# ctu-vras/monoforce

Measured on AMD Instinct MI355X. Metric: rollout-steps/sec (batch x horizon) on 256x256 terrain, higher is better.
Workload: dtype f32; 1 GPU; c3: B=1024/GPU x T=500 x N=4 contact points, 256x256 grid (res 0.05 m), one shared terrain+friction map (the same on every rank), integrator=odeint-euler (reference default), forward+backward; BASE...; rollouts_per_gpu=1024, rollouts_total=1024, horizon=500, contact_points=4, parallelism=rollout-sharded x1

## Files before the change

monoforce_amd/csrc/rollout_bwd_cp_kernel.h:

```cpp
#pragma once
#include "rollout_bwd_kernel.h"
#include "rollout_cp_common.h"
#include <type_traits>

namespace mf {

enum { kCpEarly = 0, kCpLate = 1, kCpSaved = 2, kCpStream = 3 };
#ifdef MF_STREAM_PROFILE
extern __device__ unsigned long long mf_stream_prof[16];
#define MF_PROF_T(v) const unsigned long long v = __builtin_readcyclecounter()
#define MF_PROF_ACC(name) unsigned long long name = 0
#define MF_PROF_SUM(name, t0) name += __builtin_readcyclecounter() - (t0)
#define MF_PROF_OUT(slot, val) do { if (lane == 0) atomicAdd(&mf_stream_prof[slot], (unsigned long long)(val)); } while (0)
#define MF_PROF_ADD(slot, t0) MF_PROF_OUT(slot, __builtin_readcyclecounter() - (t0))
#else
#define MF_PROF_T(v)
#define MF_PROF_ACC(name)
#define MF_PROF_SUM(name, t0)
#define MF_PROF_OUT(slot, val)
#define MF_PROF_ADD(slot, t0)
#endif
#ifdef MF_NO_WPE
#define MF_STREAM_WPE
#else
#define MF_STREAM_WPE __attribute__((amdgpu_waves_per_eu((MODE == kCpStream && XS_ONLY && sizeof(S) == 4) ? 2 : 1)))
#endif
template <typename S, int INTEG, bool XS_ONLY, bool GCTRL, int MODE, int SLOTS = 6, int BATCH = 3, bool ZMU = false, bool WIN = false, bool ONE1 = false>
__global__ void __launch_bounds__(MODE == kCpStream ? 192 : (WIN ? 512 : 256)) MF_STREAM_WPE
rollout_bwd_cp_kernel(const RolloutBwdArgs<S> a) {
  constexpr bool ODE = INTEG == MF_INTEG_ODEINT_EULER;
  constexpr bool LATE = MODE == kCpLate, STREAM = MODE == kCpStream, SAVED = MODE == kCpSaved || STREAM;
  using namespace cp;
  using M = Mth<S, std::is_same<S, float>::value>;
  using Msk = typename MaskOf<S>::type;
  constexpr unsigned kS = (unsigned)sizeof(S), kC = 2u * kS;
  const int lane = threadIdx.x & 63;
  const int tid = STREAM ? blockIdx.x * 64 + lane : blockIdx.x * blockDim.x + threadIdx.x;
  const int b = tid >> 4;
  __shared__ S win[WIN ? 2 * kWinW * kWinW : 1];
  int wx0 = 0, wy0 = 0;
  unsigned win_flat0 = 0u, win_shift = 0u;
  if constexpr (WIN) {
    static_assert(MODE != kCpStream && sizeof(S) == 4, "the LDS gradient window serves the float32 one-wave forms");
    win_open<S, true>(a, win, (int)((blockIdx.x * blockDim.x) >> 4), &wx0, &wy0);
    __syncthreads();
    win_shift = 31u - (unsigned)__builtin_clz((unsigned)a.H);
    win_flat0 = (unsigned)wy0 + ((unsigned)wx0 << win_shift);
  }
  if (b >= a.B) return;
  const int p = (tid >> 2) & 3, q = tid & 3, cc = q < 3 ? q : 2;
  const S one = S(1.0), zero = S(0.0);
  const int HW = a.H * a.W, last = HW - 1;
  const unsigned moff = a.map_shared ? 0u : (unsigned)b * (unsigned)HW;
  const S* zmap = a.z;
  const bool has_mu = a.mu != nullptr;
  const S* mumap = has_mu ? a.mu : a.z;
  const unsigned goff = a.map_shared ? (unsigned)(b % a.grad_copies) * (unsigned)HW : (unsigned)b * (unsigned)HW;
  S* gzmap = a.gz;
  const bool want_gmu = a.gmu != nullptr && has_mu;
  S* gmumap = want_gmu ? a.gmu : a.gz;

  const bool act = p < a.N;
  const int pi = act ? p : 0;
  const S P0 = a.points[pi * 3 + 0], P1 = a.points[pi * 3 + 1], P2 = a.points[pi * 3 + 2];
  const int part = act ? a.part[pi] : -1;
  const S tv_v = part < 0 ? zero : one;
  const S tv_w = part < 0 ? zero : ((part & 1) ? a.half_ly : -a.half_ly);
  const S I0 = a.Iinv[cc * 3 + 0], I1 = a.Iinv[cc * 3 + 1], I2 = a.Iinv[cc * 3 + 2];
  const S J0 = a.Iinv[0 * 3 + cc], J1 = a.Iinv[1 * 3 + cc], J2 = a.Iinv[2 * 3 + cc];
// ... 87 lines not shown
    }
  };
  const S first = p == 0 ? one : zero;
  auto add_upstream_masked = [&](const UpIn& u) {
    lx += u.gXs;
    lR2 = mf_fma(u.gXs, a.sink, lR2);
    if constexpr (!XS_ONLY) {
      lxd += u.gXds;
      lR0 += u.gR0; lR1 += u.gR1; lR2 += u.gR2;
      lw += u.gOm;
    }
  };
  auto add_upstream_state = [&](const UpIn& u) {
    UpIn m = u;
    S gXs_row = u.gXs;
    if constexpr (ONE1) {
      const Msk smask = u.lw > zero ? ~(Msk)0 : (Msk)0;
      gXs_row = bfi(smask, cp_loss_grad(one1_scale, u.gXs, u.lg, u.lw), zero);
    }
    m.gXs = first * gXs_row;
    if constexpr (!XS_ONLY) { m.gXds = first * u.gXds; m.gR0 = first * u.gR0; m.gR1 = first * u.gR1; m.gR2 = first * u.gR2; m.gOm = first * u.gOm; }
    add_upstream_masked(m);
  };

  if constexpr (GCTRL && ODE) bstore2(rGctrl, v_ctrl, (unsigned)(a.T - 1) * kC, zero, zero);

  unsigned acc_idx = 0u, st_idx = 0u;
  S acc_z = zero, acc_m = zero, st_z = zero, st_m = zero;
  bool st_pending = false;
  auto emit = [&](unsigned idx, S vz, S vm) {
    if constexpr (WIN) {
      if (win_emit(win, win_flat0, win_shift, (unsigned)(a.H - 1), idx, vz, vm, want_gmu)) return;
    }
    atomic_add(at32(gzmap, goff + idx), vz);
    if (want_gmu) atomic_add(at32(gmumap, goff + idx), vm);
  };
  auto flush_stash = [&]() {
    if (st_pending) emit(st_idx, st_z, st_m);
    st_pending = false;
  };

  unsigned gctrl_pending = (unsigned)(a.T - 1) * kC;
  S gv_pending = zero, gwc_pending = zero;

  struct Rec {
    S x, xd, cv, cw, r, pc, fr, mc;
    S R0, R1, R2, w, r1, r2, w1, w2, vp, e, il, coln2, tv, h;
    S wq, wa, wb, zc, mcv, mub, nrm, inl, cj, inv_csum, A, F0, F1, Fr, Nn, cmdv, s, sn, stv, Gf, f1, f2, wraw;
    int idx;
  };
  auto recompute_gather = [&](const StateIn& st, Rec& k) {
    k.x = st.x; k.xd = st.xd; k.w = st.w; k.cv = st.cv; k.cw = st.cw;
    k.R0 = st.R0; k.R1 = st.R1; k.R2 = st.R2;
    k.h = ODE ? st.t1 - st.t0 : a.dt;
    k.r = cp_body_r(P0, P1, P2, st.R0, st.R1, st.R2);
    k.pc = k.r + st.x;
    const S lim = S(262144.0);
    const S uq = M::cell_coord(k.pc, a.d_max, a.res, a.inv_res);
    const int ui = (int)M::clamp(uq, -lim, lim);
    k.fr = uq - (S)ui;
    const int base = dppi<kB1>(ui) + __mul24(a.H, dppi<kB0>(ui));
    k.idx = min(max(base + cell_off, 0), last);
    k.zc = ld32(zmap, moff + (unsigned)k.idx);
    k.mc = ld32(mumap, moff + (unsigned)k.idx);
  };
  auto recompute = [&](Rec& k) {
// ... 148 lines not shown
    const S gpx = dot4(vq, wa_s * k.wb), gpy = dot4(vq, wb_s * k.wa);
    const S gp = mask_or(mask_or(mask_or(zero, gpx * a.inv_res, lane0), gpy * a.inv_res, lane1), gdh, lane2);
    const S gvp1 = dpp<kRot1>(gvp), gvp2 = dpp<kRot2>(gvp);
    gr += gvp1 * w2 - gvp2 * w1;
    const S gw_p = r1 * gvp2 - r2 * gvp1;
    const S qa = gp + gr;
    lx += gp; lxd += gvp; lw += gw_p;
    lR0 = mf_fma(qa, P0, lR0); lR1 = mf_fma(qa, P1, lR1); lR2 = mf_fma(qa, P2, lR2);
    const S ge = ge_p;
    S gv = zero, gwc = zero;
    if constexpr (GCTRL) { gv = sum_points(gv_p); gwc = sum_points(gwc_p); }
    {
      const S dote = dot3(ge, k.e) * (k.coln2 >= S(1e-12) ? one : zero);
      lR0 = mf_fma(ge - dote * k.e, k.il, lR0);
    }
    gctrl_pending = __builtin_amdgcn_readfirstlane((unsigned)n * kC); gv_pending = gv; gwc_pending = gwc;
  };

  auto body = [&](int n, const Rec& rec, Rec& rec_next, const StateIn& s_prev, StateIn& s_pp, const UpIn& up, UpIn& up_next) {
    add_upstream_state(up);
    load_state(max(n - 2, 0), s_pp);
    load_upstream(ODE ? n : max(n - 1, 0), up_next);
    recompute_gather(s_prev, rec_next);
    if constexpr (!LATE) recompute(rec_next);
    flush_stash();
    if constexpr (GCTRL) bstore2(rGctrl, v_ctrl, gctrl_pending, gv_pending, gwc_pending);
    vjp(n, rec, up);
    if constexpr (LATE) {
      asm("" : "+v"(rec_next.zc), "+v"(rec_next.mc) : "v"(lR0));
      recompute(rec_next);
    }
  };

  StateIn sA, sB;
  UpIn uA, uB;
  Rec recA, recB;
  int n = n_steps - 1;
  if constexpr (SAVED) {
    typedef S f4v __attribute__((ext_vector_type(4)));
    struct Saved { f4v q; S zc, mc; int idx; };
    const char* const prec = reinterpret_cast<const char*>(a.rec) + (size_t)tid * kRecBytesPerLane<S>;
    const unsigned rec_step = (unsigned)a.B * 16u * kRecBytesPerLane<S>;
    auto load_saved = [&](int m, Saved& v) {
      v.q = __builtin_nontemporal_load(reinterpret_cast<const f4v*>(prec + (size_t)__builtin_amdgcn_readfirstlane((unsigned)m) * (size_t)rec_step));
    };
    auto gather_cells = [&](Saved& v) {
      const S lim = S(262144.0);
      const int ui = (int)M::clamp(v.q.x, -lim, lim);
      const int base = dppi<kB1>(ui) + __mul24(a.H, dppi<kB0>(ui));
      v.idx = min(max(base + cell_off, 0), last);
#ifdef MF_STREAM_NO_GATHER
      v.zc = S(0.1) * (S)q; v.mc = S(0.8);
      return;
#endif
      if constexpr (ZMU) {
        const Pk2<S> zm = *reinterpret_cast<const Pk2<S>*>(reinterpret_cast<const char*>(a.zmu) + (size_t)((unsigned)v.idx * (unsigned)(2 * sizeof(S))));
        v.zc = zm.a; v.mc = zm.b;
        return;
      }
      v.zc = ld32(zmap, moff + (unsigned)v.idx);
      v.mc = ld32(mumap, moff + (unsigned)v.idx);
    };
    auto rebuild = [&](const StateIn& st, const Saved& v, Rec& k) {
      k.R0 = st.R0; k.R1 = st.R1; k.R2 = st.R2; k.w = st.w;
      k.h = ODE ? st.t1 - st.t0 : a.dt;
      const S r = cp_body_r(P0, P1, P2, st.R0, st.R1, st.R2);
// ... 58 lines not shown
          const bool init = ti == 0;
          const unsigned p3 = init ? o3 : o3 - s3, p9 = init ? o9 : o9 - s9;
          const S xd = bload1<S>(rXds, p3, 0u), w = bload1<S>(rOm, p3, 0u);
          S R0, R1, R2;
          bload3(rRs, p9, 0u, &R0, &R1, &R2);
          d.xd = init ? ini.xd : xd; d.w = init ? ini.w : w;
          d.R0 = init ? ini.R0 : R0; d.R1 = init ? ini.R1 : R1; d.R2 = init ? ini.R2 : R2;
          d.x = bload1<S>(rOm, o3, 0u);
          d.t1 = a.dt; d.t0 = zero;
        }
        bload2(rCtrl, oc, 0u, &d.cv, &d.cw);
        v.q = __builtin_nontemporal_load(reinterpret_cast<const f4v*>(prec + (size_t)orc));
      };
      auto request_up = [&](UpIn& u) {
#ifdef MF_STREAM_NO_FETCH
        u.gXs = S(0.001);
        if constexpr (!XS_ONLY) { u.gXds = u.gOm = u.gR0 = u.gR1 = u.gR2 = u.gFs = u.gFf = S(0.001); }
        return;
#endif
        u.gXs = bload1<S>(rgXs, og_xs, 0u);
        if constexpr (!XS_ONLY) {
          u.gXds = bload1<S>(rgXds, og_xds, 0u); u.gOm = bload1<S>(rgOm, og_om, 0u);
          bload3(rgRs, og_r, 0u, &u.gR0, &u.gR1, &u.gR2);
          u.gFs = bload1<S>(rgFs, og_fs, 0u); u.gFf = bload1<S>(rgFf, og_ff, 0u);
        }
      };
      auto step_back_up = [&]() {
        og_xs -= sg_xs;
        if constexpr (!XS_ONLY) { og_xds -= sg_xds; og_om -= sg_om; og_r -= sg_r; og_fs -= sg_fs; og_ff -= sg_ff; }
      };
      constexpr int kSlots = SLOTS, kPlanesD = ODE ? 0 : 6, kPlanes = (XS_ONLY ? 10 : 12) + kPlanesD;
      constexpr bool kPow2 = (kSlots & (kSlots - 1)) == 0;
      __shared__ f4v ring[kSlots * kPlanes * 64];
      __shared__ int flags[2];
      typedef __attribute__((address_space(3))) volatile int LdsCounter;
      LdsCounter* vflags = (LdsCounter*)flags;
      if (threadIdx.x == 0) { flags[0] = 0; flags[1] = 0; }
      __syncthreads();
      const bool loss_val = loss_on && a.loss_out != nullptr;
      __shared__ S l_part[3 * 16 + 64];
      auto loss_value_finish = [&](S acc) {
        if (!loss_val) return;
        const int wv = (int)(threadIdx.x >> 6);
        if (lane < 16) l_part[wv * 16 + lane] = zero;
        if (p == 0 && q < 3) l_part[wv * 16 + (lane >> 4) * 4 + q] = acc;
        __syncthreads();
        if (wv != 0) return;
        unsigned last_wg = 0u;
        if (lane == 0) {
          S tot = zero;
#pragma unroll
          for (int r = 0; r < 4; ++r)
#pragma unroll
            for (int v = 0; v < 3; ++v) tot += (l_part[v * 16 + r * 4 + 0] + l_part[v * 16 + r * 4 + 1]) + l_part[v * 16 + r * 4 + 2];
          __builtin_nontemporal_store(tot, a.loss_partial + blockIdx.x);
          __threadfence();
          last_wg = atomicAdd(a.loss_ticket, 1u) == gridDim.x - 1 ? 1u : 0u;
        }
        last_wg = __builtin_amdgcn_readfirstlane(last_wg);
        if (last_wg) {
          __threadfence();
          const int n_act = min(64, (a.B - (int)blockIdx.x * 4) * 16);
          S tot = zero;
          for (unsigned k2 = (unsigned)lane; k2 < gridDim.x; k2 += (unsigned)n_act) tot += __builtin_nontemporal_load(a.loss_partial + k2);
          l_part[48 + lane] = tot;
          asm volatile("s_waitcnt lgkmcnt(0)" ::: "memory");
          if (lane == 0) {
            S sum = zero;
            for (int k2 = 0; k2 < n_act; ++k2) sum += l_part[48 + k2];
            a.loss_out[0] = sum * a.loss_inv_count;
            *a.loss_ticket = 0u;
          }
        }
      };
      if (threadIdx.x >= 64) {
        static_assert(kSlots % BATCH == 0 && (BATCH == 2 || BATCH == 3), "a batch must not wrap around the ring");
        struct Slot { StateIn st; Saved sv; UpIn up; S lg, lw; int sj; };
        unsigned zero_lane = 0u;
        asm("" : "+v"(zero_lane));
        const int fk = __builtin_amdgcn_readfirstlane((int)(threadIdx.x >> 6)) - 1;
        int m = n;
        S l_acc = zero;
        auto fetch = [&](Slot& r) {
          request_state(r.st, r.sv);
          request_up(r.up);
          r.sj = ld32(l_row_stamp, (unsigned)ti + kUp + zero_lane);
          r.lw = ld32(l_row_w, (unsigned)ti + kUp + zero_lane);
          r.lg = zero;
          o3 -= s3; o9 -= s9; oc -= kC; orc -= rec_step; --ti;
          step_back_up();
          --m;
        };
        constexpr unsigned kB = (unsigned)BATCH;
        auto skip3 = [&]() {
          o3 -= kB * s3; o9 -= kB * s9; oc -= kB * kC; orc -= kB * rec_step; ti -= BATCH; m -= BATCH;
          og_xs -= kB * sg_xs;
          if constexpr (!XS_ONLY) { og_xds -= kB * sg_xds; og_om -= kB * sg_om; og_r -= kB * sg_r; og_fs -= kB * sg_fs; og_ff -= kB * sg_ff; }
        };
        MF_PROF_T(t_fetcher);
        MF_PROF_ACC(acc_room); MF_PROF_ACC(acc_pub);
        auto room = [&](int upto) {
          MF_PROF_T(t0);
          while (upto - __builtin_amdgcn_readfirstlane(vflags[1]) > kSlots) __builtin_amdgcn_s_sleep(2);
          asm volatile("" ::: "memory");
          MF_PROF_SUM(acc_room, t0);
        };
        auto publish = [&](int from, int upto) {
          asm volatile("" ::: "memory");
          MF_PROF_T(t0);
          while (__builtin_amdgcn_readfirstlane(vflags[0]) != from) __builtin_amdgcn_s_sleep(1);
          asm volatile("" ::: "memory");
          MF_PROF_SUM(acc_pub, t0);
          vflags[0] = upto;
        };
        auto put = [&](const Slot& r, unsigned slot, int o) {
            Rec k;
            rebuild(r.st, r.sv, k);
            const S mw = inside(k.wraw, -a.omega_max, a.omega_max) ? one : zero;
            const S mG = inside(k.Gf, -mg, mg) ? one : zero;
            const S mF1 = inside(k.F1, -mg, mg) ? one : zero;
            const S invNn = k.Nn > zero ? M::div(one, k.Nn) : zero;
            const S cmask = k.coln2 >= S(1e-12) ? one : zero;
            const S cs = k.cj * k.inv_csum;
            const f4v p0 = f4v{k.R0, k.R1, k.R2, k.h};
            const f4v p1 = f4v{k.w1, k.w2, k.r1, k.r2};
            const f4v p2 = f4v{k.f1, k.f2, mw, mG * k.stv};
            const f4v p3 = f4v{mG * k.Nn, k.nrm, k.s, k.sn};
            const f4v p4 = f4v{k.cmdv, k.mub, k.tv * k.mub, k.Fr * invNn};
            const f4v p5 = f4v{mF1 * cs, mF1 * k.nrm, k.A, -(a.k * cs)};
            const f4v p6 = f4v{-(a.damp * cs), -(k.A * k.inv_csum), k.A * k.cj * k.inv_csum * k.inv_csum, -S(10.0) * k.cj * (one - k.cj)};
            const f4v p7 = f4v{k.vp, -(k.inl * a.inv_res), k.wq, idx_as(zero, k.idx)};
            const f4v p8 = f4v{k.zc, k.mcv, wa_s * k.wb * a.inv_res, wb_s * k.wa * a.inv_res};
            const Msk smask = r.sj >= 0 ? ~(Msk)0 : (Msk)0;
            const S gXs_row = bfi(loss_mask, bfi(smask, cp_loss_grad(loss_scale, r.up.gXs, r.lg, r.lw), zero), r.up.gXs);
            l_acc += bfi(smask, cp_loss_term(r.up.gXs, r.lg, r.lw), zero);
            const f4v p9 = f4v{k.e, k.il, cmask * k.e * k.il, first * gXs_row};
            f4v d0 = {zero, zero, zero, zero}, d1 = d0, d2 = d0, d3 = d0, d4 = d0, d5 = d0;
            if constexpr (!ODE) {
              const S h = a.dt, wn = r.st.x;
              const S th2 = dot3(wn, wn);
              const S idn = M::inv_len(th2);
              const S kv = wn * idn;
              const S th = M::sqrt(th2);
              S sn_, oc;
              M::sincos_small(th * h, &sn_, &oc);
              const S kk = dot3(kv, kv);
              const S kv1 = dpp<kRot1>(kv), kv2 = dpp<kRot2>(kv);
              const S ok = oc * kv;
              const S m0 = mf_fma(ok, kv, mf_fma(-oc, kk, one)), m1 = mf_fma(ok, kv1, -(sn_ * kv2)), m2 = mf_fma(ok, kv2, sn_ * kv1);
              const S q0 = dpp<kB0>(kv), q1 = dpp<kB1>(kv), q2 = dpp<kB2>(kv);
              const S Rk = k.R0 * q0 + k.R1 * q1 + k.R2 * q2;
              const S idn2 = th2 >= S(1e-12) ? idn * idn : zero;
              const S ith = th2 > zero ? M::div(one, th) : zero;
              d0 = f4v{wn, kv, q0, q1};
              d1 = f4v{q2, Rk, kk, sn_};
              d2 = f4v{oc, h * (one - oc), h * sn_, idn};
              d3 = f4v{idn2, ith, dpp<kB0>(m0), dpp<kB0>(m1)};
              d4 = f4v{dpp<kB0>(m2), dpp<kB1>(m2), dpp<kB1>(m0), dpp<kB1>(m1)};
              d5 = f4v{dpp<kB2>(m1), dpp<kB2>(m2), dpp<kB2>(m0), zero};
            }
            room(o + 1);
            f4v* out = ring + slot * (unsigned)(kPlanes * 64) + lane;
            out[0] = p0; out[64] = p1; out[128] = p2; out[192] = p3; out[256] = p4; out[320] = p5; out[384] = p6; out[448] = p7; out[512] = p8; out[576] = p9;
            if constexpr (!XS_ONLY) {
              out[640] = f4v{first * r.up.gXds, first * r.up.gOm, r.up.gFs, r.up.gFf};
              out[704] = f4v{first * r.up.gR0, first * r.up.gR1, first * r.up.gR2, zero};
            }
            if constexpr (!ODE) {
              constexpr int D0 = (XS_ONLY ? 10 : 12) * 64;
              out[D0] = d0; out[D0 + 64] = d1; out[D0 + 128] = d2; out[D0 + 192] = d3; out[D0 + 256] = d4; out[D0 + 320] = d5;
            }
            publish(o, o + 1);
          };
        int ord = BATCH * fk;
        unsigned sbase = kB * (unsigned)fk;
        auto fetch3 = [&](Slot (&s)[BATCH]) {
#pragma unroll
          for (int i = 0; i < BATCH; ++i) fetch(s[i]);
          skip3();
        };
        auto gather1 = [&](Slot& r) {
          gather_cells(r.sv);
          r.lg = loss_gt_lane[(size_t)(unsigned)min(max(r.sj, 0), l_T2m1) * 3u];
        };
        auto gather3 = [&](Slot (&s)[BATCH]) {
#pragma unroll
          for (int i = 0; i < BATCH; ++i) gather1(s[i]);
        };
        auto put3 = [&](const Slot (&s)[BATCH]) {
#pragma unroll
          for (int i = 0; i < BATCH; ++i) put(s[i], sbase + (unsigned)i, ord + i);
          ord += 2 * BATCH;
          if constexpr (kSlots != 2 * BATCH) sbase = sbase + 2u * kB >= (unsigned)kSlots ? sbase + 2u * kB - (unsigned)kSlots : sbase + 2u * kB;
        };
        Slot A[BATCH], B[BATCH], C[BATCH];
        const int n_full = (n + 1) / BATCH;
        int full = (n_full - fk + 1) / 2;
        if (fk == 1) skip3();
        if (full >= 2) {
          fetch3(A); fetch3(B); gather3(A);
          full -= 2;
          while (full >= 3) {
            fetch3(C); gather3(B); put3(A);
            fetch3(A); gather3(C); put3(B);
            fetch3(B); gather3(A); put3(C);
            full -= 3;
          }
          if (full == 0) { gather3(B); put3(A); put3(B); }
          else if (full == 1) { fetch3(C); gather3(B); put3(A); gather3(C); put3(B); put3(C); }
          else { fetch3(C); gather3(B); put3(A); fetch3(A); gather3(C); put3(B); gather3(A); put3(C); put3(A); }
        } else if (full == 1) { fetch3(A); gather3(A); put3(A); }
        if (fk == (n_full & 1)) {
          int o = BATCH * n_full;
          unsigned sl = sbase;
          while (m >= 0) {
            Slot r0;
            fetch(r0);
            gather1(r0);
            put(r0, sl, o);
            ++sl; ++o;
          }
        }
        MF_PROF_ADD(2 + 4 * fk, t_fetcher);
        MF_PROF_OUT(0 + 4 * fk, acc_room); MF_PROF_OUT(1 + 4 * fk, acc_pub);
        loss_value_finish(l_acc);
        return;
      }
        int consumed = 0, seen = 0;
        unsigned rslot = 0u;
        UpIn uZ;
        load_upstream(0, uZ);
        S l_row0 = zero;
        if (loss_on && ODE) {
          const S g0 = loss_gt_lane[(size_t)max(a.loss_row_stamp[0], 0) * 3u], w0 = a.loss_row_w[0];
          const bool stamped = a.loss_row_stamp[0] >= 0;
          l_row0 = stamped ? cp_loss_term(uZ.gXs, g0, w0) : zero;
          uZ.gXs = stamped ? cp_loss_grad(loss_scale, uZ.gXs, g0, w0) : zero;
        }
        struct Coef {
          S R0, R1, R2, h, w1, w2, r1, r2, f1, f2, mw;
          S stvG, NnG, nrm, s, sn;
          S cmdv, mub, tvm, FrN;
          S csm, nm1, A, kcs;
          S dcs, Aic, Acc, dcj;
          S vp, inlr, wq, zc, mcv, wsb, wsa;
          S e, il, eci;
          int idx;
          S wn, kv, q0, q1, q2, Rk, kk, sn_, oc, cga, cgb, idn, idn2, ith;
          S M00, M01, M02, M10, M11, M12, M20, M21, M22;
        };
        MF_PROF_T(t_compute);
        MF_PROF_ACC(acc_wait);
        auto ensure = [&](int k) {
          MF_PROF_T(t0);
          int have = __builtin_amdgcn_readfirstlane(seen);
          while (have < consumed + k) have = __builtin_amdgcn_readfirstlane(vflags[0]);
          asm volatile("" ::: "memory");
          MF_PROF_SUM(acc_wait, t0);
        };
        auto grab = [&](Coef& c, UpIn& up) {
          const f4v* o = ring + (kPow2 ? (unsigned)(consumed & (kSlots - 1)) : rslot) * (unsigned)(kPlanes * 64) + lane;
          if constexpr (!kPow2) rslot = rslot + 1u == (unsigned)kSlots ? 0u : rslot + 1u;
          const f4v c0 = o[0], c1 = o[64], c2 = o[128], c3 = o[192], c4 = o[256], c5 = o[320], c6 = o[384], c7 = o[448], c8 = o[512], c9 = o[576];
          const S idx_bits = c7.w;
          c.R0 = c0.x; c.R1 = c0.y; c.R2 = c0.z; c.h = c0.w;
          c.w1 = c1.x; c.w2 = c1.y; c.r1 = c1.z; c.r2 = c1.w;
          c.f1 = c2.x; c.f2 = c2.y; c.mw = c2.z; c.stvG = c2.w;
          c.NnG = c3.x; c.nrm = c3.y; c.s = c3.z; c.sn = c3.w;
          c.cmdv = c4.x; c.mub = c4.y; c.tvm = c4.z; c.FrN = c4.w;
          c.csm = c5.x; c.nm1 = c5.y; c.A = c5.z; c.kcs = c5.w;
          c.dcs = c6.x; c.Aic = c6.y; c.Acc = c6.z; c.dcj = c6.w;
          c.vp = c7.x; c.inlr = c7.y; c.wq = c7.z; c.idx = idx_of(idx_bits);
          c.zc = c8.x; c.mcv = c8.y; c.wsb = c8.z; c.wsa = c8.w;
          c.e = c9.x; c.il = c9.y; c.eci = c9.z; up.gXs = c9.w;
          if constexpr (!XS_ONLY) {
            const f4v g0 = o[640];
            const S* g1 = reinterpret_cast<const S*>(o + 704);
            up.gXds = g0.x; up.gOm = g0.y; up.gFs = g0.z; up.gFf = g0.w; up.gR0 = g1[0]; up.gR1 = g1[1]; up.gR2 = g1[2];
          }
          if constexpr (!ODE) {
            constexpr int D0 = (XS_ONLY ? 10 : 12) * 64;
            const f4v e0 = o[D0], e1 = o[D0 + 64], e2 = o[D0 + 128], e3 = o[D0 + 192], e4 = o[D0 + 256];
            const S* e5 = reinterpret_cast<const S*>(o + D0 + 320);
            c.wn = e0.x; c.kv = e0.y; c.q0 = e0.z; c.q1 = e0.w;
            c.q2 = e1.x; c.Rk = e1.y; c.kk = e1.z; c.sn_ = e1.w;
            c.oc = e2.x; c.cga = e2.y; c.cgb = e2.z; c.idn = e2.w;
            c.idn2 = e3.x; c.ith = e3.y; c.M00 = e3.z; c.M01 = e3.w;
            c.M02 = e4.x; c.M10 = e4.y; c.M11 = e4.z; c.M12 = e4.w;
            c.M20 = e5[0]; c.M21 = e5[1]; c.M22 = e5[2];
          }
          ++consumed;
// ... 92 lines not shown
          }
          const S vq = gzq * c.zc + gmuq * c.mcv;
          const S gpx = dot4(vq, c.wsb), gpy = dot4(vq, c.wsa);
          const S gp = mask_or(mask_or(mask_or(zero, gpx, lane0), gpy, lane1), gdh, lane2);
          const S gvp1 = dpp<kRot1>(gvp), gvp2 = dpp<kRot2>(gvp);
          gr += gvp1 * c.w2 - gvp2 * c.w1;
          const S gw_p = c.r1 * gvp2 - c.r2 * gvp1;
          const S qa = gp + gr;
          lx += gp; lxd += gvp; lw += gw_p;
          lR0 = mf_fma(qa, P0, lR0); lR1 = mf_fma(qa, P1, lR1); lR2 = mf_fma(qa, P2, lR2);
          S gv = zero, gwc = zero;
          if constexpr (GCTRL) { gv = sum_points(gv_p); gwc = sum_points(gwc_p); }
          lR0 = mf_fma(-dot3(ge_p, c.e), c.eci, mf_fma(ge_p, c.il, lR0));
          gctrl_pending = __builtin_amdgcn_readfirstlane((unsigned)n * kC); gv_pending = gv; gwc_pending = gwc;
        };
        auto crunch = [&](int n, const Coef& c, const UpIn& up, Coef& c_next, UpIn& up_next, auto more, auto paired) {
          add_upstream_masked(up);
          if constexpr (decltype(paired)::value == 1) grab(c_next, up_next);
          else if constexpr (decltype(paired)::value == 2) { grab(c_next, up_next); release(); }
          else if constexpr (decltype(more)::value) take(c_next, up_next);
          flush_stash();
          if constexpr (GCTRL) bstore2(rGctrl, v_ctrl, gctrl_pending, gv_pending, gwc_pending);
#ifdef MF_STREAM_NO_VJP
          asm volatile("" :: "v"(c.R0), "v"(c.w1), "v"(c.f1), "v"(c.NnG), "v"(c.cmdv), "v"(c.csm), "v"(c.dcs), "v"(c.vp), "v"(c.zc), "v"(c.e));
#else
          chain(n, c, up);
#endif
        };
        using std::true_type;
        using std::false_type;
        Coef cA, cB;
        if (n_steps > 0) {
          take(cA, uA);
          using single = std::integral_constant<int, 0>;
          for (; n >= 2; n -= 2) {
            ensure(2);
            crunch(n, cA, uA, cB, uB, true_type{}, std::integral_constant<int, 1>{});
            crunch(n - 1, cB, uB, cA, uA, true_type{}, std::integral_constant<int, 2>{});
          }
          if (n == 1) { crunch(1, cA, uA, cB, uB, true_type{}, single{}); crunch(0, cB, uB, cA, uA, false_type{}, single{}); }
          else crunch(0, cA, uA, cB, uB, false_type{}, single{});
        }
        MF_PROF_ADD(9, t_compute);
        MF_PROF_OUT(8, acc_wait);
        loss_value_finish(l_row0);
        uA = uZ; uB = uZ;
    } else {
      struct Raw { StateIn st; Saved sv; };
      Raw S_[3];
      Rec K_[3];
      UpIn U_[3];
      auto up_row = [&](int m) { return ODE ? max(m + 1, 0) : max(m, 0); };
      auto run = [&](auto rtag, int n) {
        constexpr int R = decltype(rtag)::value, R1 = (R + 1) % 3, R2 = (R + 2) % 3;
        add_upstream_state(U_[R]);
        gather_cells(S_[R1].sv);
#ifndef MF_SAVED_NO_STATE
        load_state(max(n - 3, 0), S_[R].st);
#endif
#ifndef MF_SAVED_NO_REC
        load_saved(max(n - 3, 0), S_[R].sv);
#endif
#ifndef MF_SAVED_NO_UP
        load_upstream(min(up_row(n - 2), a.T - 1), U_[R2]);
#endif
#ifndef MF_SAVED_NO_ATOMIC
        flush_stash();
#endif
        if constexpr (GCTRL) bstore2(rGctrl, v_ctrl, gctrl_pending, gv_pending, gwc_pending);
#ifndef MF_SAVED_NO_VJP
        vjp(n, K_[R], U_[R]);
#endif
#ifndef MF_SAVED_NO_VJP
        asm("" : "+v"(S_[R1].sv.zc), "+v"(S_[R1].sv.mc) : "v"(lR0));
#endif
#ifndef MF_SAVED_NO_REBUILD
        rebuild(S_[R1].st, S_[R1].sv, K_[R1]);
#endif
// ... 9 lines not shown
      load_saved(max(n0 - 2, 0), S_[2].sv);
      gather_cells(S_[0].sv);
      rebuild(S_[0].st, S_[0].sv, K_[0]);
      __builtin_amdgcn_s_waitcnt(0);
      using std::integral_constant;
      int i = 0;
      for (; i + 2 < n_steps; i += 3) {
        run(integral_constant<int, 0>{}, n0 - i);
        run(integral_constant<int, 1>{}, n0 - i - 1);
        run(integral_constant<int, 2>{}, n0 - i - 2);
      }
      if (i < n_steps) run(integral_constant<int, 0>{}, n0 - i);
      if (i + 1 < n_steps) run(integral_constant<int, 1>{}, n0 - i - 1);
      {
        const int r0 = (n0 + 1) % 3;
        uA = r0 == 0 ? U_[0] : (r0 == 1 ? U_[1] : U_[2]);
        uB = uA;
      }
      n = -1;
    }
  } else {
  load_state(max(n, 0), sA);
  load_upstream(min(max(n, 0) + (ODE ? 1 : 0), a.T - 1), uA);
  load_state(max(n - 1, 0), sB);
  recompute_gather(sA, recA);
  recompute(recA);
  __builtin_amdgcn_s_waitcnt(0);
  for (; n >= 1; n -= 2) {
    body(n, recA, recB, sB, sA, uA, uB);
    body(n - 1, recB, recA, sA, sB, uB, uA);
  }
  if (n == 0) body(0, recA, recB, sB, sA, uA, uB);
  }
  UpIn up = (n_steps & 1) ? uB : uA;
  flush_stash();
  if constexpr (GCTRL) bstore2(rGctrl, v_ctrl, gctrl_pending, gv_pending, gwc_pending);
  if (act) emit(acc_idx, acc_z, acc_m);
  if constexpr (ODE) {
    if (n_steps == 0) load_upstream(0, up);
    add_upstream_state(up);
  }
  lx = sum_points(lx); lxd = sum_points(lxd); lw = sum_points(lw);
  lR0 = sum_points(lR0); lR1 = sum_points(lR1); lR2 = sum_points(lR2);

  S gx0 = lx;
  if (!a.skip_snap) {
    const S Ra = a.R0[b * 9 + cc * 3 + 0], Rb = a.R0[b * 9 + cc * 3 + 1], Rc = a.R0[b * 9 + cc * 3 + 2];
    const S x0c = a.x_init[b * 3 + cc];
    const S g = dpp<kB2>(lx) / (S)a.N;
    const S pc = (P0 * Ra + P1 * Rb + P2 * Rc) + x0c;
    const S lim = S(262144.0);
    const S uq = M::cell_coord(pc, a.d_max, a.res, a.inv_res);
    const int ui = (int)M::clamp(uq, -lim, lim);
    const S fr = uq - (S)ui;
    const int base = dppi<kB1>(ui) + __mul24(a.H, dppi<kB0>(ui));
    const int idx = min(max(base + cell_off, 0), last);
    const S wa = mf_fma(wa_s, dpp<kB0>(fr), wa_o), wb = mf_fma(wb_s, dpp<kB1>(fr), wb_o);
    const S zc = ld32(zmap, moff + (unsigned)idx);
    if (act) atomic_add(at32(gzmap, goff + (unsigned)idx), g * (wa * wb));
    const S gpx = dot4(zc, wa_s * wb) * g * a.inv_res, gpy = dot4(zc, wb_s * wa) * g * a.inv_res;
    S gpxy = q == 0 ? gpx : (q == 1 ? gpy : zero);
    gpxy = act ? gpxy : zero;
    gx0 = (q < 2 ? lx : zero) + sum_points(gpxy);
    lR0 += sum_points(gpxy * P0); lR1 += sum_points(gpxy * P1); lR2 += sum_points(gpxy * P2);
  }
  if (p == 0) {
    if (a.gx0) a.gx0[b * 3 + cc] = gx0;
    a.gxd0[b * 3 + cc] = lxd;
    a.gw0[b * 3 + cc] = lw;
    a.gR0[b * 9 + cc * 3 + 0] = lR0; a.gR0[b * 9 + cc * 3 + 1] = lR1; a.gR0[b * 9 + cc * 3 + 2] = lR2;
  }
  if constexpr (WIN) {
    __syncthreads();
    win_close(a, win, wx0, wy0);
  }
}

bool use_component_parallel_bwd(const MfRolloutDesc* d, const MfRolloutBwdBufs* p, int scalar_bytes = 4);
long long cp_record_bytes(const MfRolloutDesc* d, int scalar_bytes);
bool cp_loss_fusable(const MfRolloutDesc* d);
bool cp_bwd_wants_zmu(const MfRolloutDesc* d, bool has_rec, bool has_mu);
int launch_rollout_bwd_cp_f32(const RolloutBwdArgs<float>& a, int integ, bool xs_only, hipStream_t st);
int launch_rollout_bwd_cp_dynamics_f32(const RolloutBwdArgs<float>& a, bool xs_only, hipStream_t st);
void launch_rollout_bwd_cp_stream_f32(const RolloutBwdArgs<float>& a, bool xs_only, unsigned grid, hipStream_t st);
void launch_rollout_bwd_cp_stream_dynamics_f32(const RolloutBwdArgs<float>& a, bool xs_only, unsigned grid, hipStream_t st);

inline unsigned cp_stream_max_grid(int integ = MF_INTEG_ODEINT_EULER) {
  static const int env = getenv("MF_CP_STREAM_MAX_GRID") ? atoi(getenv("MF_CP_STREAM_MAX_GRID")) : -1;
  const unsigned cus = (unsigned)device_cus();
  const unsigned v = env >= 0 ? (unsigned)env : 2u * cus;
  return integ == MF_INTEG_ODEINT_EULER ? v : (v < cus ? v : cus);
}

void launch_rollout_bwd_cp_stream_f64(const RolloutBwdArgs<double>& a, bool xs_only, unsigned grid, hipStream_t st);
int launch_rollout_bwd_cp_f64(const RolloutBwdArgs<double>& a, int integ, bool xs_only, hipStream_t st);
inline void launch_rollout_bwd_cp_stream_any(const RolloutBwdArgs<float>& a, int integ, bool xs_only, unsigned grid, hipStream_t st) {
  if (integ == MF_INTEG_ODEINT_EULER) launch_rollout_bwd_cp_stream_f32(a, xs_only, grid, st); else launch_rollout_bwd_cp_stream_dynamics_f32(a, xs_only, grid, st);
}
inline void launch_rollout_bwd_cp_stream_any(const RolloutBwdArgs<double>& a, int, bool xs_only, unsigned grid, hipStream_t st) {
  launch_rollout_bwd_cp_stream_f64(a, xs_only, grid, st);
}
template <typename S>
inline unsigned cp_stream_max_grid_of(int integ) {
  if (sizeof(S) == 8) return integ == MF_INTEG_ODEINT_EULER ? cp_stream_max_grid(integ) : 0u;
// ... 50 lines not shown
```

monoforce_amd/csrc/rollout_bwd_cp_stream_fast.hip:

```cpp
#include "rollout_bwd_cp_kernel.h"

#ifdef MF_STREAM_PROFILE
namespace mf { __device__ unsigned long long mf_stream_prof[16]; }
extern "C" int mf_debug_stream_profile(unsigned long long* out16, int reset) {
  if (out16) { if (hipMemcpyFromSymbol(out16, HIP_SYMBOL(mf::mf_stream_prof), sizeof(mf::mf_stream_prof)) != hipSuccess) return 1; }
  if (reset) { unsigned long long z[16] = {}; if (hipMemcpyToSymbol(HIP_SYMBOL(mf::mf_stream_prof), z, sizeof(z)) != hipSuccess) return 2; }
  return 0;
}
#endif
namespace mf {

void launch_rollout_bwd_cp_stream_f32(const RolloutBwdArgs<float>& a, bool xs_only, unsigned grid, hipStream_t st) {
  constexpr int I = MF_INTEG_ODEINT_EULER;
  const bool gc = a.gcontrols != nullptr;
  static const int big_ring_env = getenv("MF_CP_STREAM_BIG_RING_MAX_GRID") ? atoi(getenv("MF_CP_STREAM_BIG_RING_MAX_GRID")) : -1;
  const unsigned big_ring_max = big_ring_env >= 0 ? (unsigned)big_ring_env : (unsigned)device_cus();
#define MF_BCPS(XS_, GC_) do { if (grid <= big_ring_max) MF_KLAUNCH((rollout_bwd_cp_kernel<float, I, XS_, GC_, kCpStream, 12>), dim3(grid), dim3(192), 0, st, a); \
                               else MF_KLAUNCH((rollout_bwd_cp_kernel<float, I, XS_, GC_, kCpStream, 6, (XS_ ? 2 : 3)>), dim3(grid), dim3(192), 0, st, a); } while (0)
  if (xs_only) { if (gc) MF_BCPS(true, true); else MF_BCPS(true, false); }
  else         { if (gc) MF_BCPS(false, true); else MF_BCPS(false, false); }
#undef MF_BCPS
}

}
```

Measured before the change: 1.346 billion rollout-steps/s.

## Overlap stream-bwd tail work across fetcher waves and batch ring publishes

In the streaming backward kernel, the idle fetcher waves now precompute the initial-state snap cell (index, bilinear weight and slope terms) into LDS while the compute wave runs, so the compute wave only reads it at the end. The loss-value reduction no longer uses a workgroup barrier. Waves post their partials through an LDS counter, and only fetcher 0 finishes the grid-wide sum, using unrolled loads and a lane-readlane reduction in place of an LDS scan. Ring publishing is batched to one wait per batch, and profiling hooks plus a no-atomic debug switch are added. The spin-waits on LDS flags add ordering subtleties and a risk of subtle races.

```diff
diff --git a/monoforce_amd/csrc/rollout_bwd_cp_kernel.h b/monoforce_amd/csrc/rollout_bwd_cp_kernel.h
--- a/monoforce_amd/csrc/rollout_bwd_cp_kernel.h
+++ b/monoforce_amd/csrc/rollout_bwd_cp_kernel.h
@@ -7,18 +7,24 @@
 
 enum { kCpEarly = 0, kCpLate = 1, kCpSaved = 2, kCpStream = 3 };
 #ifdef MF_STREAM_PROFILE
-extern __device__ unsigned long long mf_stream_prof[16];
+extern __device__ unsigned long long mf_stream_prof[32];
 #define MF_PROF_T(v) const unsigned long long v = __builtin_readcyclecounter()
+#define MF_PROF_RT(v) const unsigned long long v = __builtin_amdgcn_s_memrealtime()
 #define MF_PROF_ACC(name) unsigned long long name = 0
 #define MF_PROF_SUM(name, t0) name += __builtin_readcyclecounter() - (t0)
 #define MF_PROF_OUT(slot, val) do { if (lane == 0) atomicAdd(&mf_stream_prof[slot], (unsigned long long)(val)); } while (0)
 #define MF_PROF_ADD(slot, t0) MF_PROF_OUT(slot, __builtin_readcyclecounter() - (t0))
+#define MF_PROF_MAX(slot, val) do { if (lane == 0) atomicMax(&mf_stream_prof[slot], (unsigned long long)(val)); } while (0)
+#define MF_PROF_DRAIN() asm volatile("s_waitcnt vmcnt(0) lgkmcnt(0)" ::: "memory")
 #else
 #define MF_PROF_T(v)
+#define MF_PROF_RT(v)
 #define MF_PROF_ACC(name)
 #define MF_PROF_SUM(name, t0)
 #define MF_PROF_OUT(slot, val)
 #define MF_PROF_ADD(slot, t0)
+#define MF_PROF_MAX(slot, val)
+#define MF_PROF_DRAIN()
 #endif
 #ifdef MF_NO_WPE
 #define MF_STREAM_WPE
@@ -35,6 +41,7 @@
   using Msk = typename MaskOf<S>::type;
   constexpr unsigned kS = (unsigned)sizeof(S), kC = 2u * kS;
   const int lane = threadIdx.x & 63;
+  MF_PROF_T(t_k0); MF_PROF_RT(rt_k0);
   const int tid = STREAM ? blockIdx.x * 64 + lane : blockIdx.x * blockDim.x + threadIdx.x;
   const int b = tid >> 4;
   __shared__ S win[WIN ? 2 * kWinW * kWinW : 1];
@@ -188,6 +195,10 @@
     if constexpr (WIN) {
       if (win_emit(win, win_flat0, win_shift, (unsigned)(a.H - 1), idx, vz, vm, want_gmu)) return;
     }
+#ifdef MF_STREAM_NO_ATOMIC
+    asm volatile("" :: "v"(vz), "v"(vm), "v"(idx));
+    return;
+#endif
     atomic_add(at32(gzmap, goff + idx), vz);
     if (want_gmu) atomic_add(at32(gmumap, goff + idx), vm);
   };
@@ -402,6 +413,24 @@
     }
   };
 
+  auto snap_cell = [&](int& idx, S& wq, S& dx, S& dy) {
+    const S Ra = a.R0[b * 9 + cc * 3 + 0], Rb = a.R0[b * 9 + cc * 3 + 1], Rc = a.R0[b * 9 + cc * 3 + 2];
+    const S x0c = a.x_init[b * 3 + cc];
+    const S pc = (P0 * Ra + P1 * Rb + P2 * Rc) + x0c;
+    const S lim = S(262144.0);
+    const S uq = M::cell_coord(pc, a.d_max, a.res, a.inv_res);
+    const int ui = (int)M::clamp(uq, -lim, lim);
+    const S fr = uq - (S)ui;
+    const int base = dppi<kB1>(ui) + __mul24(a.H, dppi<kB0>(ui));
+    idx = min(max(base + cell_off, 0), last);
+    const S wa = mf_fma(wa_s, dpp<kB0>(fr), wa_o), wb = mf_fma(wb_s, dpp<kB1>(fr), wb_o);
+    const S zc = ld32(zmap, moff + (unsigned)idx);
+    wq = wa * wb;
+    dx = dot4(zc, wa_s * wb); dy = dot4(zc, wb_s * wa);
+  };
+  int snap_idx = 0;
+  S snap_wq = zero, snap_dx = zero, snap_dy = zero;
+
   StateIn sA, sB;
   UpIn uA, uB;
   Rec recA, recB;
@@ -526,20 +555,25 @@
       constexpr int kSlots = SLOTS, kPlanesD = ODE ? 0 : 6, kPlanes = (XS_ONLY ? 10 : 12) + kPlanesD;
       constexpr bool kPow2 = (kSlots & (kSlots - 1)) == 0;
       __shared__ f4v ring[kSlots * kPlanes * 64];
-      __shared__ int flags[2];
+      __shared__ int flags[4];
       typedef __attribute__((address_space(3))) volatile int LdsCounter;
       LdsCounter* vflags = (LdsCounter*)flags;
-      if (threadIdx.x == 0) { flags[0] = 0; flags[1] = 0; }
+      if (threadIdx.x == 0) { flags[0] = 0; flags[1] = 0; flags[2] = 0; flags[3] = 0; }
       __syncthreads();
       const bool loss_val = loss_on && a.loss_out != nullptr;
-      __shared__ S l_part[3 * 16 + 64];
-      auto loss_value_finish = [&](S acc) {
+      __shared__ S l_part[3 * 16];
+      auto loss_share = [&](S acc) {
         if (!loss_val) return;
         const int wv = (int)(threadIdx.x >> 6);
         if (lane < 16) l_part[wv * 16 + lane] = zero;
         if (p == 0 && q < 3) l_part[wv * 16 + (lane >> 4) * 4 + q] = acc;
-        __syncthreads();
-        if (wv != 0) return;
+        asm volatile("" ::: "memory");
+        if (lane == 0) __hip_atomic_fetch_add(&flags[2], 1, __ATOMIC_RELAXED, __HIP_MEMORY_SCOPE_WORKGROUP);
+      };
+      auto loss_value_finish = [&]() {
+        if (!loss_val) return;
+        while (__builtin_amdgcn_readfirstlane(vflags[2]) != 3) __builtin_amdgcn_s_sleep(1);
+        asm volatile("" ::: "memory");
         unsigned last_wg = 0u;
         if (lane == 0) {
           S tot = zero;
@@ -556,16 +590,36 @@
           __threadfence();
           const int n_act = min(64, (a.B - (int)blockIdx.x * 4) * 16);
           S tot = zero;
-          for (unsigned k2 = (unsigned)lane; k2 < gridDim.x; k2 += (unsigned)n_act) tot += __builtin_nontemporal_load(a.loss_partial + k2);
-          l_part[48 + lane] = tot;
-          asm volatile("s_waitcnt lgkmcnt(0)" ::: "memory");
+          for (unsigned k0 = (unsigned)lane; k0 < gridDim.x; k0 += 8u * (unsigned)n_act) {
+            S v[8];
+#pragma unroll
+            for (int i = 0; i < 8; ++i) {
+              const unsigned k2 = k0 + (unsigned)(i * n_act);
+              v[i] = __builtin_nontemporal_load(a.loss_partial + min(k2, gridDim.x - 1u));
+              v[i] = k2 < gridDim.x ? v[i] : zero;
+            }
+#pragma unroll
+            for (int i = 0; i < 8; ++i) tot += v[i];
+          }
+          S sum = zero;
+#pragma unroll
+          for (int k2 = 0; k2 < 64; ++k2) sum += k2 < n_act ? mf_readlane(tot, k2) : zero;
           if (lane == 0) {
-            S sum = zero;
-            for (int k2 = 0; k2 < n_act; ++k2) sum += l_part[48 + k2];
             a.loss_out[0] = sum * a.loss_inv_count;
             *a.loss_ticket = 0u;
           }
         }
+      };
+      __shared__ S snap_c[4 * 64];
+      auto snap_prepare = [&]() {
+        if (!a.skip_snap) {
+          S wq, dx, dy;
+          int idx;
+          snap_cell(idx, wq, dx, dy);
+          snap_c[lane] = idx_as(zero, idx); snap_c[64 + lane] = wq; snap_c[128 + lane] = dx; snap_c[192 + lane] = dy;
+        }
+        asm volatile("" ::: "memory");
+        vflags[3] = 1;
       };
       if (threadIdx.x >= 64) {
         static_assert(kSlots % BATCH == 0 && (BATCH == 2 || BATCH == 3), "a batch must not wrap around the ring");
@@ -599,13 +653,20 @@
           asm volatile("" ::: "memory");
           MF_PROF_SUM(acc_room, t0);
         };
-        auto publish = [&](int from, int upto) {
+        int pub = 0;
+        auto publish_written = [&](int upto) {
+          asm volatile("" ::: "memory");
+          if (__builtin_amdgcn_readfirstlane(vflags[0]) == pub) { vflags[0] = upto; pub = upto; }
+        };
+        auto publish = [&](int upto) {
           asm volatile("" ::: "memory");
           MF_PROF_T(t0);
-          while (__builtin_amdgcn_readfirstlane(vflags[0]) != from) __builtin_amdgcn_s_sleep(1);
-          asm volatile("" ::: "memory");
+          if (pub != upto) {
+            while (__builtin_amdgcn_readfirstlane(vflags[0]) != pub) __builtin_amdgcn_s_sleep(1);
+            asm volatile("" ::: "memory");
+            vflags[0] = upto; pub = upto;
+          }
           MF_PROF_SUM(acc_pub, t0);
-          vflags[0] = upto;
         };
         auto put = [&](const Slot& r, unsigned slot, int o) {
             Rec k;
@@ -664,7 +725,10 @@
               constexpr int D0 = (XS_ONLY ? 10 : 12) * 64;
               out[D0] = d0; out[D0 + 64] = d1; out[D0 + 128] = d2; out[D0 + 192] = d3; out[D0 + 256] = d4; out[D0 + 320] = d5;
             }
-            publish(o, o + 1);
+            publish_written(o + 1);
+#ifdef MF_STREAM_PROFILE
+            if (o == 0) MF_PROF_ADD(18, t_k0);
+#endif
           };
         int ord = BATCH * fk;
         unsigned sbase = kB * (unsigned)fk;
@@ -682,8 +746,10 @@
           for (int i = 0; i < BATCH; ++i) gather1(s[i]);
         };
         auto put3 = [&](const Slot (&s)[BATCH]) {
+          pub = ord;
 #pragma unroll
           for (int i = 0; i < BATCH; ++i) put(s[i], sbase + (unsigned)i, ord + i);
+          publish(ord + BATCH);
           ord += 2 * BATCH;
           if constexpr (kSlots != 2 * BATCH) sbase = sbase + 2u * kB >= (unsigned)kSlots ? sbase + 2u * kB - (unsigned)kSlots : sbase + 2u * kB;
         };
@@ -711,13 +777,27 @@
             Slot r0;
             fetch(r0);
             gather1(r0);
+            pub = o;
             put(r0, sl, o);
+            publish(o + 1);
             ++sl; ++o;
           }
         }
         MF_PROF_ADD(2 + 4 * fk, t_fetcher);
         MF_PROF_OUT(0 + 4 * fk, acc_room); MF_PROF_OUT(1 + 4 * fk, acc_pub);
-        loss_value_finish(l_acc);
+        loss_share(l_acc);
+        if (fk == 0) {
+          MF_PROF_T(t_lf);
+          loss_value_finish();
+          MF_PROF_DRAIN();
+          MF_PROF_ADD(21, t_lf);
+#ifdef MF_STREAM_PROFILE
+          MF_PROF_MAX(17, __builtin_readcyclecounter() - t_lf);
+          MF_PROF_MAX(14, __builtin_amdgcn_s_memrealtime());
+#endif
+        } else {
+          snap_prepare();
+        }
         return;
       }
         int consumed = 0, seen = 0;
@@ -731,6 +811,7 @@
           l_row0 = stamped ? cp_loss_term(uZ.gXs, g0, w0) : zero;
           uZ.gXs = stamped ? cp_loss_grad(loss_scale, uZ.gXs, g0, w0) : zero;
         }
+        loss_share(l_row0);
         struct Coef {
           S R0, R1, R2, h, w1, w2, r1, r2, f1, f2, mw;
           S stvG, NnG, nrm, s, sn;
@@ -745,12 +826,21 @@
         };
         MF_PROF_T(t_compute);
         MF_PROF_ACC(acc_wait);
+#ifdef MF_STREAM_PROFILE
+        unsigned long long acc_wait_early = 0, acc_wait_late = 0, n_waited = 0;
+#endif
         auto ensure = [&](int k) {
           MF_PROF_T(t0);
           int have = __builtin_amdgcn_readfirstlane(seen);
           while (have < consumed + k) have = __builtin_amdgcn_readfirstlane(vflags[0]);
           asm volatile("" ::: "memory");
           MF_PROF_SUM(acc_wait, t0);
+#ifdef MF_STREAM_PROFILE
+          const unsigned long long dt = __builtin_readcyclecounter() - t0;
+          if (consumed < 30) acc_wait_early += dt;
+          if (consumed >= n_steps - 30) acc_wait_late += dt;
+          n_waited += __builtin_amdgcn_readfirstlane(seen) < consumed + k ? 1u : 0u;
+#endif
         };
         auto grab = [&](Coef& c, UpIn& up) {
           const f4v* o = ring + (kPow2 ? (unsigned)(consumed & (kSlots - 1)) : rslot) * (unsigned)(kPlanes * 64) + lane;
@@ -909,6 +999,7 @@
         Coef cA, cB;
         if (n_steps > 0) {
           take(cA, uA);
+          MF_PROF_ADD(3, t_k0); MF_PROF_OUT(19, acc_wait);
           using single = std::integral_constant<int, 0>;
           for (; n >= 2; n -= 2) {
             ensure(2);
@@ -920,7 +1011,19 @@
         }
         MF_PROF_ADD(9, t_compute);
         MF_PROF_OUT(8, acc_wait);
-        loss_value_finish(l_row0);
+#ifdef MF_STREAM_PROFILE
+        MF_PROF_OUT(22, acc_wait_early); MF_PROF_OUT(23, n_waited); MF_PROF_OUT(24, acc_wait_late);
+#endif
+        MF_PROF_ADD(20, t_k0);
+        MF_PROF_DRAIN();
+        MF_PROF_T(t_sw);
+        if (!a.skip_snap) {
+          while (__builtin_amdgcn_readfirstlane(vflags[3]) == 0) __builtin_amdgcn_s_sleep(1);
+          asm volatile("" ::: "memory");
+          snap_idx = idx_of(snap_c[lane]); snap_wq = snap_c[64 + lane]; snap_dx = snap_c[128 + lane]; snap_dy = snap_c[192 + lane];
+        }
+        MF_PROF_DRAIN();
+        MF_PROF_ADD(7, t_sw);
         uA = uZ; uB = uZ;
     } else {
       struct Raw { StateIn st; Saved sv; };
@@ -996,6 +1099,7 @@
   }
   if (n == 0) body(0, recA, recB, sB, sA, uA, uB);
   }
+  MF_PROF_T(t_e0);
   UpIn up = (n_steps & 1) ? uB : uA;
   flush_stash();
   if constexpr (GCTRL) bstore2(rGctrl, v_ctrl, gctrl_pending, gv_pending, gwc_pending);
@@ -1006,23 +1110,16 @@
   }
   lx = sum_points(lx); lxd = sum_points(lxd); lw = sum_points(lw);
   lR0 = sum_points(lR0); lR1 = sum_points(lR1); lR2 = sum_points(lR2);
+  MF_PROF_DRAIN();
+  MF_PROF_ADD(10, t_e0);
+  MF_PROF_T(t_s0);
 
   S gx0 = lx;
   if (!a.skip_snap) {
-    const S Ra = a.R0[b * 9 + cc * 3 + 0], Rb = a.R0[b * 9 + cc * 3 + 1], Rc = a.R0[b * 9 + cc * 3 + 2];
-    const S x0c = a.x_init[b * 3 + cc];
+    if constexpr (!STREAM) snap_cell(snap_idx, snap_wq, snap_dx, snap_dy);
     const S g = dpp<kB2>(lx) / (S)a.N;
-    const S pc = (P0 * Ra + P1 * Rb + P2 * Rc) + x0c;
-    const S lim = S(262144.0);
-    const S uq = M::cell_coord(pc, a.d_max, a.res, a.inv_res);
-    const int ui = (int)M::clamp(uq, -lim, lim);
-    const S fr = uq - (S)ui;
-    const int base = dppi<kB1>(ui) + __mul24(a.H, dppi<kB0>(ui));
-    const int idx = min(max(base + cell_off, 0), last);
-    const S wa = mf_fma(wa_s, dpp<kB0>(fr), wa_o), wb = mf_fma(wb_s, dpp<kB1>(fr), wb_o);
-    const S zc = ld32(zmap, moff + (unsigned)idx);
-    if (act) atomic_add(at32(gzmap, goff + (unsigned)idx), g * (wa * wb));
-    const S gpx = dot4(zc, wa_s * wb) * g * a.inv_res, gpy = dot4(zc, wb_s * wa) * g * a.inv_res;
+    if (act) atomic_add(at32(gzmap, goff + (unsigned)snap_idx), g * snap_wq);
+    const S gpx = snap_dx * g * a.inv_res, gpy = snap_dy * g * a.inv_res;
     S gpxy = q == 0 ? gpx : (q == 1 ? gpy : zero);
     gpxy = act ? gpxy : zero;
     gx0 = (q < 2 ? lx : zero) + sum_points(gpxy);
@@ -1034,6 +1131,16 @@
     a.gw0[b * 3 + cc] = lw;
     a.gR0[b * 9 + cc * 3 + 0] = lR0; a.gR0[b * 9 + cc * 3 + 1] = lR1; a.gR0[b * 9 + cc * 3 + 2] = lR2;
   }
+#ifdef MF_STREAM_PROFILE
+  if constexpr (STREAM) {
+    MF_PROF_DRAIN();
+    MF_PROF_ADD(11, t_s0);
+    MF_PROF_RT(rt_end);
+    MF_PROF_ADD(12, t_k0);
+    MF_PROF_MAX(13, __builtin_readcyclecounter() - t_k0);
+    MF_PROF_MAX(14, rt_end); MF_PROF_MAX(15, ~rt_k0); MF_PROF_OUT(16, rt_end - rt_k0);
+  }
+#endif
   if constexpr (WIN) {
     __syncthreads();
     win_close(a, win, wx0, wy0);
diff --git a/monoforce_amd/csrc/rollout_bwd_cp_stream_fast.hip b/monoforce_amd/csrc/rollout_bwd_cp_stream_fast.hip
--- a/monoforce_amd/csrc/rollout_bwd_cp_stream_fast.hip
+++ b/monoforce_amd/csrc/rollout_bwd_cp_stream_fast.hip
@@ -1,10 +1,10 @@
 #include "rollout_bwd_cp_kernel.h"
 
 #ifdef MF_STREAM_PROFILE
-namespace mf { __device__ unsigned long long mf_stream_prof[16]; }
-extern "C" int mf_debug_stream_profile(unsigned long long* out16, int reset) {
-  if (out16) { if (hipMemcpyFromSymbol(out16, HIP_SYMBOL(mf::mf_stream_prof), sizeof(mf::mf_stream_prof)) != hipSuccess) return 1; }
-  if (reset) { unsigned long long z[16] = {}; if (hipMemcpyToSymbol(HIP_SYMBOL(mf::mf_stream_prof), z, sizeof(z)) != hipSuccess) return 2; }
+namespace mf { __device__ unsigned long long mf_stream_prof[32]; }
+extern "C" int mf_debug_stream_profile(unsigned long long* out32, int reset) {
+  if (out32) { if (hipMemcpyFromSymbol(out32, HIP_SYMBOL(mf::mf_stream_prof), sizeof(mf::mf_stream_prof)) != hipSuccess) return 1; }
+  if (reset) { unsigned long long z[32] = {}; if (hipMemcpyToSymbol(HIP_SYMBOL(mf::mf_stream_prof), z, sizeof(z)) != hipSuccess) return 2; }
   return 0;
 }
 #endif
```

After: 1.380 billion rollout-steps/s (median of 6 runs). 2.5% higher.
